# GAP-LAB-CUHK-SZ/GaussReg

Hardware: AMD Instinct MI355X
Metric: GS views/sec @1M pts 640x480 (+ radius_neighbors Mpts/sec, see radius_neighbors) (higher is better)
Workload: dtype f32; 1 GPU; diff_gaussian_rasterization forward: 1000000 synthetic Gaussians (SH deg 3), 640x480, 32 views per step per GPU (configs[1]); gaussians=1000000, width=640, height=480, parallelism=per-view sharding x1

## Files before the change

### gaussreg_amd/_lib.py

```python
import ctypes
import os
import re

_HERE = os.path.dirname(os.path.abspath(__file__))
LIB_PATH = os.path.join(_HERE, "lib", "libgaussreg_hip.so")
HEADER_PATH = os.path.join(_HERE, "..", "include", "gaussreg_hip.h")
TRAIN_HEADER_PATH = os.path.join(_HERE, "..", "include", "gaussreg_hip_train.h")
MATCH_TRAIN_HEADER_PATH = os.path.join(_HERE, "..", "include", "gaussreg_hip_train_matching.h")
BACKBONE_TRAIN_HEADER_PATH = os.path.join(_HERE, "..", "include", "gaussreg_hip_train_backbone.h")
CLOUD_HEADER_PATH = os.path.join(_HERE, "..", "include", "gaussreg_hip_cloud.h")
ICP_HEADER_PATH = os.path.join(_HERE, "..", "include", "gaussreg_hip_icp.h")

_lib = None

c_void = ctypes.c_void_p
c_f32 = ctypes.c_float


class RasterView(ctypes.Structure):
    _fields_ = [("image_height", ctypes.c_int32), ("image_width", ctypes.c_int32),
                ("tanfovx", c_f32), ("tanfovy", c_f32), ("bg", c_f32 * 3), ("scale_modifier", c_f32),
                ("viewmatrix", c_f32 * 16), ("projmatrix", c_f32 * 16), ("campos", c_f32 * 3),
                ("sh_degree", ctypes.c_int32), ("prefiltered", ctypes.c_int32), ("debug", ctypes.c_int32)]


class GsAdamGroup(ctypes.Structure):
    _fields_ = [("param", c_void), ("grad", c_void), ("exp_avg", c_void), ("exp_avg_sq", c_void),
                ("lr", ctypes.c_double), ("K", ctypes.c_int32)]


class GsDensifyGroup(ctypes.Structure):
    _fields_ = [("src_param", c_void), ("dst_param", c_void), ("src_exp_avg", c_void), ("dst_exp_avg", c_void),
                ("src_exp_avg_sq", c_void), ("dst_exp_avg_sq", c_void), ("K", ctypes.c_int32), ("role", ctypes.c_int32)]


_SCALARS = {"int": ctypes.c_int, "int32_t": ctypes.c_int32, "uint32_t": ctypes.c_uint32, "int64_t": ctypes.c_int64,
            "size_t": ctypes.c_size_t, "float": ctypes.c_float, "double": ctypes.c_double}
_POINTEES = set(_SCALARS) | {"void", "uint8_t", "uint64_t"}
_STRUCTS = {"gr_raster_view": RasterView, "gr_gs_adam_group": GsAdamGroup, "gr_gs_densify_group": GsDensifyGroup}
_TYPE = r"(?:const\s+)?(\w+)"


def _ctype(base, star, where):
    if star:
        if base == "char":
            return ctypes.c_char_p
        if base in _STRUCTS:
            return ctypes.POINTER(_STRUCTS[base])
        if base in _POINTEES:
            return ctypes.c_void_p
    elif base in _SCALARS:
        return _SCALARS[base]
    raise ValueError(f"gaussreg_hip.h: type '{base}{star}' in {where} is outside the binding's vocabulary")


def parse_header(text):
    text = re.sub(r"/\*.*?\*/", " ", text, flags=re.S)
    defines = {m.group(1): int(m.group(2)) for m in re.finditer(r"^[ \t]*#[ \t]*define[ \t]+(GR_\w+)[ \t]+(-?\d+)[ \t]*$",
                                                                  text, flags=re.M)}
    text = re.sub(r"^[ \t]*#.*$", "", text, flags=re.M)
    text = re.sub(r"\b(?:typedef\s+struct|enum)\b[^{};]*\{[^{}]*\}[^;]*;", "", text)
    text = re.sub(r'extern\s+"C"\s*\{(.*)\}', r"\1", text, flags=re.S)
    signatures = {}
    for decl in filter(None, (" ".join(d.split()) for d in text.split(";"))):
        m = re.fullmatch(r"(.+?)\b(gr_\w+) ?\((.*)\)", decl)
        if m is None:
            raise ValueError(f"gaussreg_hip.h: cannot parse the declaration '{decl}'")
        ret, name, args = m.group(1).strip(), m.group(2), m.group(3).strip()
        r = re.fullmatch(_TYPE + r"\s*(\*?)", ret)
        if r is None:
            raise ValueError(f"gaussreg_hip.h: cannot parse the return type '{ret}' of {name}")
        restype = None if r.groups() == ("void", "") else _ctype(r.group(1), r.group(2), f"the return type of {name}")
        argtypes = []
        for arg in ([] if args in ("", "void") else args.split(",")):
            a = re.fullmatch(_TYPE + r"(?:\s*(\*)\s*|\s+)\w+", arg.strip())
            if a is None:
                raise ValueError(f"gaussreg_hip.h: cannot parse the argument '{arg.strip()}' of {name}")
            argtypes.append(_ctype(a.group(1), a.group(2) or "", f"argument '{arg.strip()}' of {name}"))
        if name in signatures:
            raise ValueError(f"gaussreg_hip.h: {name} is declared twice")
        signatures[name] = (restype, argtypes)
    return signatures, defines


with open(HEADER_PATH) as _f:
    SIGNATURES, DEFINES = parse_header(_f.read())
with open(TRAIN_HEADER_PATH) as _f:
    TRAIN_SIGNATURES, TRAIN_DEFINES = parse_header(_f.read())
with open(MATCH_TRAIN_HEADER_PATH) as _f:
    MATCH_TRAIN_SIGNATURES, MATCH_TRAIN_DEFINES = parse_header(_f.read())
with open(BACKBONE_TRAIN_HEADER_PATH) as _f:
    BACKBONE_TRAIN_SIGNATURES, BACKBONE_TRAIN_DEFINES = parse_header(_f.read())
with open(CLOUD_HEADER_PATH) as _f:
    CLOUD_SIGNATURES, CLOUD_DEFINES = parse_header(_f.read())
with open(ICP_HEADER_PATH) as _f:
    ICP_SIGNATURES, ICP_DEFINES = parse_header(_f.read())

GR_PENDING = DEFINES["GR_PENDING"]
GR_RETRY_FULL = DEFINES["GR_RETRY_FULL"]
GR_RETRY_BIN = DEFINES["GR_RETRY_BIN"]
GS_ADAM_MAX_GROUPS = DEFINES["GR_GS_ADAM_MAX_GROUPS"]
GS_KNN_MAX_K = DEFINES["GR_GS_KNN_MAX_K"]
CLOUD_KNN_MAX_K = CLOUD_DEFINES["GR_CLOUD_KNN_MAX_K"]
CLOUD_ICP_MAX_ITERATIONS = ICP_DEFINES["GR_CLOUD_ICP_MAX_ITERATIONS"]
GS_DENSIFY_CARRIED, GS_DENSIFY_XYZ, GS_DENSIFY_SCALING = (DEFINES["GR_GS_DENSIFY_" + r] for r in ("CARRIED", "XYZ", "SCALING"))


class HipLibraryError(RuntimeError):
    pass


def lib():
    global _lib
    if _lib is None:
        import torch
        if not os.path.exists(LIB_PATH):
            raise HipLibraryError(
                f"{LIB_PATH} is missing: build it with `python -m gaussreg_amd.build` "
                "(there is no CPU fallback for the gaussreg_amd ops)")
        L = ctypes.CDLL(LIB_PATH)
        for name, (res, args) in (list(SIGNATURES.items()) + list(TRAIN_SIGNATURES.items())
                                   + list(MATCH_TRAIN_SIGNATURES.items()) + list(BACKBONE_TRAIN_SIGNATURES.items())
                                   + list(CLOUD_SIGNATURES.items()) + list(ICP_SIGNATURES.items())):
            fn = getattr(L, name)
            fn.restype = res
            fn.argtypes = args
        _lib = L
    return _lib


def check(rc, allow=()):
    if rc != 0 and rc not in allow:
        msg = lib().gr_last_error()
        raise RuntimeError("gaussreg_hip: " + (msg.decode() if msg else f"error {rc}"))
    return rc


def tensor_stamp(tensors):
    out = []
    for t in tensors:
        if t.is_inference():
            return None
        out.append((t.data_ptr(), t._version))
    return tuple(out)


def require_gpu():
    import torch
    if not torch.cuda.is_available():
        raise HipLibraryError("gaussreg_amd ops need an MI355X (torch.cuda.is_available() is False); "
                              "there is no CPU fallback")
    return torch.device("cuda", torch.cuda.current_device())


_ws_cache = {}


def workspace(device, nbytes):
    import threading

    import torch
    key = (device.type, device.index, torch.cuda.current_stream(device).cuda_stream, threading.get_ident())
    buf = _ws_cache.get(key)
    if buf is None or buf.numel() < nbytes:
        buf = torch.empty(int(nbytes * 1.25) + 4096, dtype=torch.uint8, device=device)
        _ws_cache[key] = buf
    return buf


def stream_ptr(device):
    import torch
    return ctypes.c_void_p(torch.cuda.current_stream(device).cuda_stream)


def ptr(t):
    return ctypes.c_void_p(t.data_ptr()) if t is not None else ctypes.c_void_p(0)
# ... 57 lines not shown
```

### gaussreg_amd/build.py

```python
import concurrent.futures
import os
import subprocess
import sys

HERE = os.path.dirname(os.path.abspath(__file__))
CSRC = os.path.join(HERE, "csrc")
LIBDIR = os.path.join(HERE, "lib")
OBJDIR = os.path.join(LIBDIR, "obj")
LIB = os.path.join(LIBDIR, "libgaussreg_hip.so")

HIPCC = os.environ.get("HIPCC", "/opt/rocm/bin/hipcc")
FLAGS = ["--offload-arch=gfx950", "-O3", "-std=c++17", "-fPIC", "-ffp-contract=off", "-Wall",
         "-Wno-unused-function", "-Wno-unused-result"]


def sources():
    return sorted(f for f in os.listdir(CSRC) if f.endswith(".hip"))


def _stale(out, deps):
    if not os.path.exists(out):
        return True
    t = os.path.getmtime(out)
    return any(os.path.getmtime(d) > t for d in deps)


def build(force=False, verbose=False):
    os.makedirs(OBJDIR, exist_ok=True)
    headers = [os.path.join(CSRC, f) for f in os.listdir(CSRC) if f.endswith((".hpp", ".h"))]
    headers += [os.path.join(HERE, "..", "include", h) for h in ("gaussreg_hip.h", "gaussreg_hip_train.h",
                                                                 "gaussreg_hip_train_matching.h",
                                                                 "gaussreg_hip_train_backbone.h", "gaussreg_hip_cloud.h",
                                                                 "gaussreg_hip_icp.h")]
    jobs = []
    objs = []
    for src in sources():
        s = os.path.join(CSRC, src)
        o = os.path.join(OBJDIR, src[:-4] + ".o")
        objs.append(o)
        if force or _stale(o, [s] + headers):
            jobs.append([HIPCC] + FLAGS + ["-c", s, "-o", o])

    def run(cmd):
        if verbose:
            print(" ".join(cmd), flush=True)
        r = subprocess.run(cmd, stdout=subprocess.PIPE, stderr=subprocess.STDOUT, text=True)
        return cmd, r.returncode, r.stdout

    if jobs:
        with concurrent.futures.ThreadPoolExecutor(max_workers=min(8, len(jobs))) as ex:
            for cmd, rc, out in ex.map(run, jobs):
                if rc != 0:
                    raise RuntimeError("hipcc failed: %s\n%s" % (" ".join(cmd), out))
                if verbose and out.strip():
                    print(out)
    if force or jobs or _stale(LIB, objs):
        cmd = [HIPCC, "--offload-arch=gfx950", "-shared", "-fPIC", "-o", LIB] + objs
        _, rc, out = run(cmd)
        if rc != 0:
            raise RuntimeError("link failed:\n" + out)
    return LIB


if __name__ == "__main__":
    print(build(force="--force" in sys.argv, verbose=True))
```

### gaussreg_amd/csrc/rasterizer.hip

```cpp
#include <algorithm>
#include <type_traits>
#include <vector>

#include <atomic>

#include "raster_shared.hpp"

namespace gr {
namespace {

static_assert(TILE == RASTER_TILE, "get_rect / rect_decode (common.hpp) are written for this tile size");


constexpr int KEY_DEPTH_BITS = 27;
constexpr uint32_t KEY_DEPTH_BASE = 0x3E000000u;

__device__ __forceinline__ uint32_t pack_rect(const int* rmin, const int* rmax) {
  const int w = rmax[0] - rmin[0], h = rmax[1] - rmin[1];
  if (w > 63 || h > 63 || rmin[0] > 126 || rmin[1] > 126) return RECT_MARKER26;
  return (uint32_t)rmin[0] | ((uint32_t)rmin[1] << 7) | ((uint32_t)w << 14) | ((uint32_t)h << 20);
}

constexpr int REC_PLANE = 66;
constexpr int SH_ROW = 13;

template <bool HAS_SH, bool HAS_COV, bool SH16, bool LATE>
__global__ __launch_bounds__(256) void preprocess_kernel(
    int P, int D, int M, int V, const DevView* __restrict__ views, const float* __restrict__ means3D,
    const float* __restrict__ shs, const float* __restrict__ colors_precomp,
    const float* __restrict__ opacities, const float* __restrict__ scales,
    const float* __restrict__ rotations, const float* __restrict__ cov3D_precomp, int W, int H,
    int32_t* __restrict__ radii, float4* __restrict__ rec, uint32_t* __restrict__ dfield,
    uint32_t* __restrict__ rect_raw, int32_t* __restrict__ far_flag, DevView cam1, int far_seq,
    int2* __restrict__ key_mm) {
  constexpr bool WAVE_MM = false;
#define GR_PREPROCESS_BODY_OK
#include "preprocess_body.hpp"
#undef GR_PREPROCESS_BODY_OK
}

template <bool HAS_SH, bool HAS_COV, bool SH16>
__global__ __launch_bounds__(256) void preprocess_many_kernel(
    int P, int D, int M, int V, const DevView* __restrict__ views, const float* __restrict__ means3D,
    const float* __restrict__ shs, const float* __restrict__ colors_precomp,
    const float* __restrict__ opacities, const float* __restrict__ scales,
    const float* __restrict__ rotations, const float* __restrict__ cov3D_precomp, int W, int H,
    int32_t* __restrict__ radii, float4* __restrict__ rec, uint32_t* __restrict__ dfield,
    uint32_t* __restrict__ rect_raw, int32_t* __restrict__ far_flag, DevView cam1, int far_seq,
    int2* __restrict__ key_mm) {
  constexpr bool WAVE_MM = true;
  constexpr bool LATE = false;
#define GR_PREPROCESS_BODY_OK
#include "preprocess_body.hpp"
#undef GR_PREPROCESS_BODY_OK
}

__global__ __launch_bounds__(256) void full_keys_kernel(int64_t n, const float4* __restrict__ rec,
                                                        const int32_t* __restrict__ radii, uint32_t* __restrict__ dfield) {
  const int64_t o = (int64_t)blockIdx.x * blockDim.x + threadIdx.x;
// ... 262 lines not shown
      int sum = 0, mx = 0;
      for (int i = threadIdx.x; i < nchunk; i += TT) {
        const int t = self.chunk_total[v * nchunk + i];
        sum += t;
        mx = max(mx, t);
      }
      sum = wave_sum_i32_dpp(sum);
      mx = wave_max_i32_dpp(mx);
      if (lane == 0) s_red[0][wv] = sum, s_red[1][wv] = mx;
      __syncthreads();
      if (threadIdx.x == 0) {
        int tv = 0, mv = 0;
        for (int w2 = 0; w2 < TT / WAVE; ++w2) tv += s_red[0][w2], mv = max(mv, s_red[1][w2]);
        self.totals[v] = tv;
        self.totals[V + v] = mv;
        if (self.mail != nullptr) {
          __hip_atomic_store(&self.mail[v], tv, __ATOMIC_RELAXED, __HIP_MEMORY_SCOPE_SYSTEM);
          __hip_atomic_store(&self.mail[V + v], mv, __ATOMIC_RELAXED, __HIP_MEMORY_SCOPE_SYSTEM);
          if (v == 0) __hip_atomic_store(&self.mail[2 * V], self.totals[2 * V], __ATOMIC_RELAXED, __HIP_MEMORY_SCOPE_SYSTEM);
          __hip_atomic_store(&self.mail[2 * V + 1 + v], self.mail_seq, __ATOMIC_RELEASE, __HIP_MEMORY_SCOPE_SYSTEM);
        }
      }
    }
  } else if (SEG == SEG_SELF_SCAN) {
    unsigned int front = (unsigned int)self.chunk_total[(int64_t)V * nchunk + v * nchunk + c];
    for (int u = 0; u < v; ++u) front += (unsigned int)self.totals[u];
    chunk_begin = front;
    total = self.chunk_total[v * nchunk + c];
  } else {
    chunk_begin = seg[0];
    total = (int)(seg[tiles] - chunk_begin);
    if (total == 0 || seg[tiles] > list_cap) return;
  }
  if (SELF && total == 0) {
    for (int T = threadIdx.x; T <= tiles; T += TT) seg[T] = chunk_begin;
    return;
  }
  const bool big = total > 0xffff;
  const bool staged = !big && total <= stage_cap;
  unsigned int* myw = s_cur + wv * (row / 2);
  unsigned short* const cur16 = reinterpret_cast<unsigned short*>(s_cur);
  unsigned short* my16 = cur16 + wv * row;
  unsigned short* stage = reinterpret_cast<unsigned short*>(s_cur + NW * (row / 2));
  unsigned int* elist = s_cur + NW * (row / 2) + (stage_cap + 1) / 2 + wv * elist_cap;
  for (int T = threadIdx.x; T < NW * (row / 2); T += TT) s_cur[T] = 0u;
  __syncthreads();
  const int w_end = min(nv, w_begin + CW);
#pragma unroll
  for (int j = 0; j < CW / WAVE; ++j) {
    const int t = w_begin + j * WAVE + lane;
    rr[j] = t < w_end ? rr[j] : 0u;
    ii[j] = t < w_end ? ii[j] : 0;
  }
  auto count = [&](int tile) { atomicAdd(&myw[tile >> 1], 1u << ((tile & 1) * 16)); };
#pragma unroll
  for (int j = 0; j < CW / WAVE; ++j) {
    const uint32_t r = rr[j];
    int x0 = 0, y0 = 0, w = 0, h = 0;
    if (r != 0u && !rect_decode(r, ii[j], vbase, rec, gx, gy, x0, y0, w, h)) w = h = 0;
    const int Mx = wave_max_i32_dpp(w), My = wave_max_i32_dpp(h);
    auto cwalk = [&](auto mtag) {
      constexpr int MX = decltype(mtag)::value;
      const int x0m = mod_small(x0, MX), y0m = mod_small(y0, My);
#pragma unroll 1
      for (int ry = 0; ry < My; ++ry) {
        int dy = ry - y0m;
        dy += dy < 0 ? My : 0;
        const int rowbase = (y0 + dy) * gx + x0;
#pragma unroll
        for (int rx = 0; rx < MX; ++rx) {
          int dx = rx - x0m;
          dx += dx < 0 ? MX : 0;
          if (dy < h && dx < w) count(rowbase + dx);
        }
      }
    };
    if (Mx == 0) continue;
    if (TT == WIDE_T || max(Mx, My) > 8) {
      for (int y = y0; y < y0 + h; ++y)
        for (int x = x0; x < x0 + w; ++x) count(y * gx + x);
    } else
      by_modulus(Mx, cwalk);
  }
  __syncthreads();
  if (SELF) {
    if (threadIdx.x == 0) s_carry = 0u;
    __syncthreads();
    for (int T0 = 0; T0 < tiles; T0 += TT) {
      const int T = T0 + (int)threadIdx.x;
      unsigned int cw[NW];
      int n_all = 0;
#pragma unroll
      for (int w2 = 0; w2 < NW; ++w2) {
        cw[w2] = T < tiles ? cur16[w2 * row + T] : 0u;
        n_all += (int)cw[w2];
      }
      const int incl = wave_incl_scan_add_dpp(n_all);
      if (lane == WAVE - 1) s_red[0][wv] = incl;
      __syncthreads();
      unsigned int before = s_carry + (unsigned int)(incl - n_all);
      for (int w2 = 0; w2 < wv; ++w2) before += (unsigned int)s_red[0][w2];
      if (T < tiles) {
        seg[T] = chunk_begin + before;
        unsigned int run = big ? 0u : before;
#pragma unroll
        for (int w2 = 0; w2 < NW; ++w2) {
          cur16[w2 * row + T] = (unsigned short)run;
          run += cw[w2];
        }
      }
      __syncthreads();
      if (threadIdx.x == TT - 1) s_carry = before + (unsigned int)n_all;
      __syncthreads();
    }
    if (threadIdx.x == 0) seg[tiles] = chunk_begin + (unsigned int)total;
    if (chunk_begin + (unsigned int)total > list_cap) return;
  } else {
    for (int T = threadIdx.x; T < tiles; T += TT) {
      unsigned int run = big ? 0u : seg[T] - chunk_begin;
#pragma unroll
      for (int w2 = 0; w2 < NW; ++w2) {
        const unsigned int n = cur16[w2 * row + T];
        cur16[w2 * row + T] = (unsigned short)run;
        run += n;
      }
    }
  }
  __syncthreads();
  auto put = [&](unsigned int tile, unsigned int pos, int local, int val) {
    if (staged) stage[pos] = (unsigned short)local;
    else if (!big) point_list[chunk_begin + pos] = val;
    else point_list[seg[tile] + pos] = val;
  };
  auto bump_raw = [&](unsigned int tile) -> unsigned int {
    return atomicAdd(&myw[tile >> 1], 1u << ((tile & 1u) * 16u));
// ... 547 lines not shown

int upload_views(const gr_raster_view* h_views, int num_views, int32_t* d_flag, hipStream_t stream) {
  static_assert(sizeof(DevView) % 4 == 0, "DevView is copied word by word");
  if (num_views <= VIEW_PACK) {
    ViewPack pack;
    memset(&pack, 0, sizeof(pack));
    for (int v = 0; v < num_views; ++v) fill_view(pack.v[v], h_views[v]);
    hipLaunchKernelGGL(upload_views_kernel, dim3(1), dim3(WAVE), 0, stream, pack, num_views, d_flag);
    GR_LAUNCH_CHECK();
    return GR_OK;
  }
  char* raw = static_cast<char*>(pinned_scratch(0, 16 + sizeof(DevView) * num_views));
  GR_REQUIRE(raw != nullptr, "pinned staging buffer for %d views could not be allocated", num_views);
  memset(raw, 0, 16);
  DevView* stage = reinterpret_cast<DevView*>(raw + 16);
  for (int v = 0; v < num_views; ++v) fill_view(stage[v], h_views[v]);
  GR_HIP(hipMemcpyAsync(d_flag, raw, 16 + sizeof(DevView) * num_views, hipMemcpyHostToDevice, stream));
  return GR_OK;
}

}
}

using namespace gr;

static int64_t tiles_of(int width, int height) {
  return (int64_t)((width + TILE - 1) / TILE) * ((height + TILE - 1) / TILE);
}

extern "C" int gr_raster_lds_atomics_lane_ordered(void) { return lds_atomics_lane_ordered_state(); }
extern "C" int gr_raster_ballot_ranking(int on) { return lds_ballot_ranking_force(on); }

extern "C" size_t gr_raster_geom_bytes(int64_t P, int num_views, int width, int height) {
  if (P < 0 || num_views < 1 || width <= 0 || height <= 0) return 0;
  return carve_geom(nullptr, P, num_views, tiles_of(width, height)).bytes;
}

extern "C" int gr_raster_debug_geom_layout(int64_t P, int num_views, int width, int height, int64_t* h_offsets) {
  GR_REQUIRE(P >= 0 && num_views >= 1 && width > 0 && height > 0 && h_offsets != nullptr, "bad argument");
  char* const origin = reinterpret_cast<char*>(uintptr_t(1) << 32);
  const Geom g = carve_geom(origin, P, num_views, tiles_of(width, height));
  h_offsets[0] = reinterpret_cast<char*>(g.dfield) - origin;
  h_offsets[1] = reinterpret_cast<char*>(g.order_b) - origin;
  h_offsets[2] = reinterpret_cast<char*>(g.rects) - origin;
  h_offsets[3] = reinterpret_cast<char*>(g.nvis) - origin;
  return 4;
}

extern "C" size_t gr_raster_bin_bytes(int64_t total_rendered, int width, int height, int num_views) {
  if (total_rendered < 0 || width <= 0 || height <= 0 || num_views < 1) return 0;
  return carve_bin(nullptr, total_rendered, tiles_of(width, height) * num_views).bytes;
}

struct Deferred {
  hipEvent_t ev;
  volatile int32_t* mail;
  int seq;
  int far_seq;
  bool by_mail;
  bool bucket_sort;
  bool self_seg;
};

static int preprocess_impl(int64_t P, int M, const float* means3D, const float* shs,
                           const float* colors_precomp, const float* opacities,
                           const float* scales, const float* rotations,
                           const float* cov3D_precomp, const gr_raster_view* h_views,
                           int num_views, int32_t* radii, void* geom, size_t geom_bytes,
                           int64_t* h_num_rendered, hipStream_t stream, Deferred* defer_ev) {
  int rc = check_views(h_views, num_views);
  if (rc != GR_OK) return rc;
  GR_REQUIRE(h_num_rendered != nullptr, "h_num_rendered is null");
  for (int v = 0; v <= num_views; ++v) h_num_rendered[v] = 0;
  GR_REQUIRE(P >= 0 && P < (1ll << 31) - 1, "P out of range");
  if (P == 0) {
    Geom g0 = carve_geom(geom, 0, num_views, tiles_of(h_views[0].image_width, h_views[0].image_height));
    if (!geom || geom_bytes < g0.bytes) {
      set_error("raster geometry buffer too small: need %zu bytes, got %zu", g0.bytes, geom_bytes);
      return GR_ERR_WORKSPACE;
    }
    rc = upload_views(h_views, num_views, g0.totals + 2 * num_views, stream);
    if (rc != GR_OK) return rc;
    GR_HIP(hipStreamSynchronize(stream));
    return GR_OK;
  }
  GR_REQUIRE(means3D && opacities && radii, "means3D / opacities / radii must be non-null");
  GR_REQUIRE((shs != nullptr) != (colors_precomp != nullptr),
             "Please provide excatly one of either SHs or precomputed colors!");
  GR_REQUIRE(((scales != nullptr && rotations != nullptr) != (cov3D_precomp != nullptr)) &&
                 ((scales != nullptr) == (rotations != nullptr)),
             "Please provide exactly one of either scale/rotation pair or precomputed 3D covariance!");
  const int D = h_views[0].sh_degree;
  if (shs) GR_REQUIRE(M >= (D + 1) * (D + 1), "shs has %d coefficients, sh_degree %d needs %d", M, D, (D + 1) * (D + 1));
  const int W = h_views[0].image_width, H = h_views[0].image_height;
  const int gx = (W + TILE - 1) / TILE, gy = (H + TILE - 1) / TILE;
  const int tiles = gx * gy;
  GR_REQUIRE(gx <= 255 && gy <= 255, "image too large: at most 255 x 255 tiles of 16 px (got %d x %d)", gx, gy);
  const size_t bin_lds = (size_t)(BIN_T / WAVE) * tiles * sizeof(unsigned int);
  GR_REQUIRE(bin_lds <= 156 * 1024, "image too large: the per-wave tile cursors (%zu bytes) do not fit in LDS", bin_lds);
  Geom g = carve_geom(geom, P, num_views, tiles);
  if (!geom || geom_bytes < g.bytes) {
    set_error("raster geometry buffer too small: need %zu bytes, got %zu", g.bytes, geom_bytes);
    return GR_ERR_WORKSPACE;
  }
  const dim3 blk(256), grd((unsigned)((P + 255) / 256));
  const bool sh16 = shs != nullptr && M == 16 && (reinterpret_cast<uintptr_t>(shs) % 16 == 0);
  const bool cam_in_args = sh16 && num_views == 1 && defer_ev != nullptr && defer_ev->mail != nullptr &&
                           (P + BIN_CHUNK - 1) / BIN_CHUNK <= SCAN_SINGLE_ROW;
  DevView cam1;
  memset(&cam1, 0, sizeof(cam1));
  int far_seq = 1;
  if (sh16 && num_views == 1) fill_view(cam1, h_views[0]);
  if (cam_in_args) {
    far_seq = defer_ev->seq;
  } else {
    rc = upload_views(h_views, num_views, g.totals + 2 * num_views, stream);
    if (rc != GR_OK) return rc;
  }
  if (defer_ev != nullptr) defer_ev->far_seq = far_seq;
  const bool msd_possible = depth_sort_msd_possible(P, num_views, KEY_DEPTH_BITS);
  const bool msd = msd_possible && (defer_ev != nullptr ? defer_ev->bucket_sort : bucket_sort_allowed(true));
  int2* const mm_out = msd ? g.key_mm : nullptr;
#define GR_PRE(SH, COV, S16)                                                                       \
  if (S16 && num_views == 1)                                                                       \
    hipLaunchKernelGGL((preprocess_kernel<SH, COV, S16, S16>), grd, blk, 0, stream, (int)P, D, M, num_views, \
                       g.views, means3D, shs, colors_precomp, opacities, scales, rotations,        \
                       cov3D_precomp, W, H, radii, g.rec, g.dfield, g.rect_raw, g.totals + 2 * num_views, cam1, far_seq, \
                       mm_out);                                                                    \
  else if (msd && num_views > 4)                                                                   \
    hipLaunchKernelGGL((preprocess_many_kernel<SH, COV, S16>), grd, blk, 0, stream, (int)P, D, M, num_views, \
                       g.views, means3D, shs, colors_precomp, opacities, scales, rotations,        \
                       cov3D_precomp, W, H, radii, g.rec, g.dfield, g.rect_raw, g.totals + 2 * num_views, cam1, far_seq, \
                       mm_out);                                                                    \
  else                                                                                             \
  hipLaunchKernelGGL((preprocess_kernel<SH, COV, S16, false>), grd, blk, 0, stream, (int)P, D, M, num_views, \
                     g.views, means3D, shs, colors_precomp, opacities, scales, rotations,          \
                     cov3D_precomp, W, H, radii, g.rec, g.dfield, g.rect_raw, g.totals + 2 * num_views, cam1, far_seq, \
                     mm_out)
  auto run_preprocess = [&]() {
    KernelTimer timer("raster_preprocess", stream);
    if (shs && cov3D_precomp) { if (sh16) GR_PRE(true, true, true); else GR_PRE(true, true, false); }
    else if (shs) { if (sh16) GR_PRE(true, false, true); else GR_PRE(true, false, false); }
    else if (cov3D_precomp) GR_PRE(false, true, false);
    else GR_PRE(false, false, false);
  };
  run_preprocess();
  GR_LAUNCH_CHECK();
  int32_t* tot = static_cast<int32_t*>(pinned_scratch(1, sizeof(int32_t) * (2 * num_views + 2)));
  GR_REQUIRE(tot != nullptr, "pinned read-back buffer could not be allocated");
  const int nchunk = (int)((P + BIN_CHUNK - 1) / BIN_CHUNK);
  int32_t h_chunk_max = 0;
  auto sort_and_count = [&](int key_bits, bool buckets = true) -> int {
    bool totals_sorted = false;
    {
      KernelTimer timer("raster_depth_sort", stream);
      const bool msd_now = msd && buckets && key_bits == KEY_DEPTH_BITS;
      const bool self_seg = msd_now && defer_ev != nullptr && defer_ev->mail != nullptr && nchunk <= SCAN_SINGLE_ROW &&
                            num_views <= 4;
      totals_sorted = msd_now && num_views > 4;
      const DepthSortTotals ct{g.chunk_total, BIN_CHUNK, nchunk, g.rec, gx, gy};
      int rcs = depth_sort_views(g.dfield, g.rect_raw, g.keys_a, g.keys_b, g.order_b, g.rects, g.nvis, P, num_views, key_bits,
                                 g.ds_table, g.ds_table_bytes, stream, msd_now ? g.key_mm : nullptr,
                                 num_views > 4 ? (int)((P + 255) / 256) * (256 / WAVE) : (int)((P + 255) / 256),
                                 g.totals + 2 * num_views, defer_ev != nullptr ? -far_seq : 2,
                                 self_seg || totals_sorted ? &ct : nullptr);
      if (rcs != GR_OK) return rcs;
      if (self_seg) {
        defer_ev->by_mail = true;
        defer_ev->self_seg = true;
        return GR_OK;
      }
    }
    {
      KernelTimer timer("raster_bin", stream);
      const bool short_rows = nchunk <= SCAN_SINGLE_ROW;
      if (!bin_scans_self(nchunk, num_views)) {
        if (tiles * sizeof(unsigned int) > 64 * 1024)
          GR_HIP(hipFuncSetAttribute(reinterpret_cast<const void*>(tile_count_kernel),
                                     hipFuncAttributeMaxDynamicSharedMemorySize, 160 * 1024));
        hipLaunchKernelGGL(tile_count_kernel, dim3((unsigned)bin_grid(num_views, nchunk)), dim3(BIN_T),
                           tiles * sizeof(unsigned int), stream, (int)P, num_views, gx, gy, nchunk, g.nvis, g.rects, g.order_b,
                           g.rec, g.chunk_cnt, g.chunk_total);
        const bool by_mail = defer_ev != nullptr && defer_ev->mail != nullptr;
        hipLaunchKernelGGL(seg_scan_kernel<true>, dim3((unsigned)(num_views * nchunk)), blk, 0, stream, num_views, tiles, nchunk,
                           g.chunk_cnt, g.chunk_total, g.totals, g.seg_off, by_mail ? const_cast<int32_t*>(defer_ev->mail) : nullptr,
                           by_mail ? defer_ev->seq : 0);
        if (by_mail) defer_ev->by_mail = true;
        GR_LAUNCH_CHECK();
      } else {
        if (!totals_sorted)
          hipLaunchKernelGGL(chunk_total_kernel, dim3((unsigned)bin_grid(num_views, nchunk)), dim3(BIN_T), 0, stream, (int)P,
                             num_views, gx, gy, nchunk, g.nvis, g.rects, g.order_b, g.rec, g.chunk_total);
        if (!short_rows)
          hipLaunchKernelGGL(chunk_max_kernel, dim3(1), dim3(1024), 0, stream, num_views * nchunk, g.chunk_total, g.chunk_max);
        GR_LAUNCH_CHECK();
        int rcs = exclusive_scan_i32(g.chunk_total, g.chunk_total + (int64_t)num_views * nchunk, nchunk, num_views, nchunk,
                                     g.scan_ws, g.totals, stream, nullptr, short_rows ? g.totals + num_views : nullptr);
        if (rcs != GR_OK) return rcs;
      }
    }
    const bool short_rows = nchunk <= SCAN_SINGLE_ROW;
    if (defer_ev != nullptr) {
      if (defer_ev->by_mail) return GR_OK;
      static thread_local hipStream_t side = nullptr;
      static thread_local hipEvent_t counted = nullptr;
      if (side == nullptr) GR_HIP(hipStreamCreateWithFlags(&side, hipStreamNonBlocking));
      if (counted == nullptr) GR_HIP(hipEventCreateWithFlags(&counted, hipEventDisableTiming));
      GR_HIP(hipEventRecord(counted, stream));
      GR_HIP(hipStreamWaitEvent(side, counted, 0));
      GR_HIP(hipMemcpyAsync(tot, g.totals, sizeof(int32_t) * (2 * num_views + 1), hipMemcpyDeviceToHost, side));
      if (!short_rows)
        GR_HIP(hipMemcpyAsync(tot + 2 * num_views + 1, g.chunk_max, sizeof(int32_t), hipMemcpyDeviceToHost, side));
      GR_HIP(hipEventRecord(defer_ev->ev, side));
      return GR_OK;
    }
    GR_HIP(hipMemcpyAsync(tot, g.totals, sizeof(int32_t) * (2 * num_views + 1), hipMemcpyDeviceToHost, stream));
    if (!short_rows)
      GR_HIP(hipMemcpyAsync(tot + 2 * num_views + 1, g.chunk_max, sizeof(int32_t), hipMemcpyDeviceToHost, stream));
    GR_HIP(hipStreamSynchronize(stream));
    h_chunk_max = short_rows ? tot[num_views] : tot[2 * num_views + 1];
    if (short_rows)
      for (int v = 1; v < num_views; ++v) h_chunk_max = std::max(h_chunk_max, tot[num_views + v]);
    return GR_OK;
  };
  rc = sort_and_count(KEY_DEPTH_BITS);
  if (rc != GR_OK) return rc;
  if (defer_ev != nullptr) return GR_OK;
  auto check_depth_order = [&]() -> int {
    if (!verify_this_frame()) return GR_OK;
    int h_bad = 0;
    int rcv = device_check(stream, [&](int* d_bad) {
      hipLaunchKernelGGL(verify_depth_order_kernel, dim3((unsigned)std::min<int64_t>((P + 255) / 256, 4096), num_views), blk, 0,
                         stream, (int)P, num_views, g.nvis, g.dfield, g.order_b, reinterpret_cast<int32_t*>(g.keys_a), d_bad);
    }, &h_bad);
    if (rcv != GR_OK) return rcv;
    if (h_bad != 0 && lds_atomics_lane_ordered_state() == 1) {
      lds_order_demote();
      return 1;
    }
    GR_REQUIRE(h_bad == 0, "depth sort produced an unsorted order (internal error)");
    return GR_OK;
  };
  if (tot[2 * num_views] & 2) {
    bucket_sort_overflowed();
    GR_HIP(hipMemsetD32Async(reinterpret_cast<hipDeviceptr_t>(g.totals + 2 * num_views), tot[2 * num_views] & 1, 1, stream));
    rc = sort_and_count(KEY_DEPTH_BITS, false);
    if (rc != GR_OK) return rc;
  }
  if (tot[2 * num_views] != 0) {
    hipLaunchKernelGGL(full_keys_kernel, dim3((unsigned)((P * num_views + 255) / 256)), blk, 0, stream, P * num_views,
                       g.rec, radii, g.dfield);
    GR_LAUNCH_CHECK();
    rc = sort_and_count(32);
    if (rc != GR_OK) return rc;
  }
  rc = check_depth_order();
  if (rc == 1) {
    rc = sort_and_count(tot[2 * num_views] != 0 ? 32 : KEY_DEPTH_BITS, false);
    if (rc != GR_OK) return rc;
    rc = check_depth_order();
// ... 165 lines not shown
  hipLaunchKernelGGL((blend_kernel<FE, KEEP>), dim3(gx, gy, num_views), dim3(BLOCK), blend_pad, stream, (int)P, W, H,      \
                     blend_chunks, g.views, g.seg_off, point_list, g.rec, out_color, list_cap, BlendAux<false>{})
#define GR_BLEND_AUX(FE, KEEP)                                                                                        \
  hipLaunchKernelGGL((blend_kernel<FE, KEEP, true>), dim3(gx, gy, num_views), dim3(BLOCK), 0, stream, (int)P, W, H,        \
                     blend_chunks, g.views, g.seg_off, point_list, g.rec, out_color, list_cap,                           \
                     BlendAux<true>{out_depth, out_alpha, aux_state})
  if (out_depth != nullptr) {
    if (keep) { if (fast) GR_BLEND_AUX(true, true); else GR_BLEND_AUX(false, true); }
    else if (fast) GR_BLEND_AUX(true, false); else GR_BLEND_AUX(false, false);
  }
  else if (keep) { if (fast) GR_BLEND(true, true); else GR_BLEND(false, true); }
  else if (fast) GR_BLEND(true, false); else GR_BLEND(false, false);
#undef GR_BLEND
#undef GR_BLEND_AUX
  GR_LAUNCH_CHECK();
  frame_done();
  return GR_OK;
}

extern "C" int gr_raster_render_ex(int64_t P, const gr_raster_view* h_views, int num_views,
                                   const int64_t* h_num_rendered, const void* geom, size_t geom_bytes,
                                   void* bin, size_t bin_bytes, float* out_color, int flags, void* stream_) {
  return render_impl(P, h_views, num_views, h_num_rendered, geom, geom_bytes, bin, bin_bytes, out_color, flags, -1,
                     static_cast<hipStream_t>(stream_));
}

extern "C" int gr_raster_render_keep(int64_t P, const gr_raster_view* h_views, int num_views,
                                     const int64_t* h_num_rendered, const void* geom, size_t geom_bytes,
                                     void* bin, size_t bin_bytes, float* out_state, int flags, void* stream_) {
  return render_impl(P, h_views, num_views, h_num_rendered, geom, geom_bytes, bin, bin_bytes, out_state, flags, -1,
                     static_cast<hipStream_t>(stream_), nullptr, true);
}

extern "C" int gr_raster_render_aux(int64_t P, const gr_raster_view* h_views, int num_views,
                                    const int64_t* h_num_rendered, const void* geom, size_t geom_bytes,
                                    void* bin, size_t bin_bytes, float* out_color, float* out_depth, float* out_alpha,
                                    float* out_state, int flags, void* stream_) {
  GR_REQUIRE(out_depth != nullptr && out_alpha != nullptr, "out_depth / out_alpha is null");
  return render_impl(P, h_views, num_views, h_num_rendered, geom, geom_bytes, bin, bin_bytes, out_color, flags, -1,
                     static_cast<hipStream_t>(stream_), nullptr, out_state != nullptr, out_depth, out_alpha, out_state);
}

namespace gr {
namespace {
struct Pending {
  bool open;
  int64_t P;
  int num_views;
  int64_t entries;
  Deferred d;
  hipStream_t stream;
};
thread_local Pending g_pending{false, 0, 0, 0, Deferred{nullptr, nullptr, 0, 0, false, false, false}, nullptr};
}
}

extern "C" int gr_raster_debug_bucket_cooldown(int set) {
  const int left = gr::g_bucket_cooldown;
  if (set >= 0) gr::g_bucket_cooldown = set;
  return left;
}

extern "C" int gr_raster_forward_finish(int64_t* h_num_rendered) {
  using namespace gr;
  GR_REQUIRE(g_pending.open, "gr_raster_forward_finish: no split gr_raster_forward is open on this thread");
  GR_REQUIRE(h_num_rendered != nullptr, "h_num_rendered is null");
  Pending p = g_pending;
  g_pending.open = false;
  bool far_depth = false, bucket_overflow = false;
  int rc = preprocess_collect(p.P, p.num_views, h_num_rendered, &far_depth, p.d, p.stream, &bucket_overflow);
  if (rc != GR_OK) return rc;
  if (bucket_overflow) bucket_sort_overflowed();
  int64_t R = 0;
  for (int v = 0; v < p.num_views; ++v) R += h_num_rendered[v];
  if (far_depth) return GR_RETRY_FULL;
  return R <= p.entries ? GR_OK : GR_RETRY_BIN;
}

extern "C" int gr_raster_forward(int64_t P, int M, const float* means3D, const float* shs, const float* colors_precomp,
                                 const float* opacities, const float* scales, const float* rotations,
                                 const float* cov3D_precomp, const gr_raster_view* h_views, int num_views, int32_t* radii,
                                 void* geom, size_t geom_bytes, void* bin, size_t bin_bytes, float* out_color, int flags,
                                 int64_t* h_num_rendered, void* stream_) {
  hipStream_t stream = static_cast<hipStream_t>(stream_);
  GR_REQUIRE(h_num_rendered != nullptr, "h_num_rendered is null");
  GR_REQUIRE(!g_pending.open, "gr_raster_forward: the previous split call of this thread was not finished");
  const int64_t stage_hint = h_num_rendered[num_views > 0 ? num_views : 0];
  const int64_t entries = bin && bin_bytes > 512 ? (int64_t)((bin_bytes - 512) / sizeof(int32_t)) - 64 : -1;
  if (P > 0 && num_views <= 4 && entries > 0 && entries < (1ll << 31) - 1 && !verify_this_frame()) {
    static thread_local hipEvent_t ev = nullptr;
    if (ev == nullptr) GR_HIP(hipEventCreateWithFlags(&ev, hipEventDisableTiming));
    static thread_local int32_t* mail = nullptr;
    if (mail == nullptr) {
      static const bool no_mail = getenv("GR_NO_MAILBOX") && getenv("GR_NO_MAILBOX")[0] == '1';
      void* mp = nullptr;
      if (!no_mail && hipHostMalloc(&mp, 4096, hipHostMallocMapped | hipHostMallocCoherent) == hipSuccess) {
        memset(mp, 0, 4096);
        mail = static_cast<int32_t*>(mp);
      } else {
        (void)hipGetLastError();
      }
    }
    static std::atomic<int> frame_seq{0};
    int seq = frame_seq.fetch_add(1) + 1;
    if (seq > 0x7ffffff0) {
      frame_seq.store(1);
      seq = 1;
    }
    Deferred d{ev, mail, seq, 1, false, bucket_sort_allowed(depth_sort_msd_possible(P, num_views, KEY_DEPTH_BITS)), false};
    int rc = preprocess_impl(P, M, means3D, shs, colors_precomp, opacities, scales, rotations, cov3D_precomp, h_views,
                             num_views, radii, geom, geom_bytes, h_num_rendered, stream, &d);
    if (rc != GR_OK) return rc;
    h_num_rendered[num_views] = stage_hint;
    rc = render_impl(P, h_views, num_views, h_num_rendered, geom, geom_bytes, bin, bin_bytes, out_color, flags, entries, stream,
                     &d);
    if (rc != GR_OK) return rc;
    if (flags & GR_RASTER_SPLIT) {
      g_pending = Pending{true, P, num_views, entries, d, stream};
      return GR_PENDING;
    }
    bool far_depth = false, bucket_overflow = false;
    rc = preprocess_collect(P, num_views, h_num_rendered, &far_depth, d, stream, &bucket_overflow);
    if (rc != GR_OK) return rc;
    if (bucket_overflow) bucket_sort_overflowed();
    int64_t R = 0;
    for (int v = 0; v < num_views; ++v) R += h_num_rendered[v];
    if (!far_depth) return R <= entries ? GR_OK : GR_RETRY_BIN;
  }
  int rc = gr_raster_preprocess(P, M, means3D, shs, colors_precomp, opacities, scales, rotations, cov3D_precomp, h_views,
                                num_views, radii, geom, geom_bytes, h_num_rendered, stream);
  if (rc != GR_OK) return rc;
  int64_t R = 0;
  for (int v = 0; v < num_views; ++v) R += h_num_rendered[v];
  if (bin == nullptr || bin_bytes < gr_raster_bin_bytes(R, h_views[0].image_width, h_views[0].image_height, num_views))
    return GR_RETRY_BIN;
  return gr_raster_render_ex(P, h_views, num_views, h_num_rendered, geom, geom_bytes, bin, bin_bytes, out_color, flags, stream);
}

extern "C" int gr_raster_mark_visible(int64_t P, const float* means3D, const float* h_viewmatrix,
                                      uint8_t* present, void* stream_) {
  hipStream_t stream = static_cast<hipStream_t>(stream_);
  GR_REQUIRE(P >= 0 && h_viewmatrix != nullptr, "bad argument");
  if (P == 0) return GR_OK;
  GR_REQUIRE(means3D && present, "null argument");
  hipLaunchKernelGGL(mark_visible_kernel, dim3((unsigned)((P + 255) / 256)), dim3(256), 0, stream, (int)P, means3D,
                     h_viewmatrix[2], h_viewmatrix[6], h_viewmatrix[10], h_viewmatrix[14], present);
  GR_LAUNCH_CHECK();
  return GR_OK;
}
```

Measured before the change: 14160 views/s.

## Extend speculative single-sync forward path to batches of more than four views

```diff
diff --git a/gaussreg_amd/_lib.py b/gaussreg_amd/_lib.py
--- a/gaussreg_amd/_lib.py
+++ b/gaussreg_amd/_lib.py
@@ -10,6 +10,7 @@
 BACKBONE_TRAIN_HEADER_PATH = os.path.join(_HERE, "..", "include", "gaussreg_hip_train_backbone.h")
 CLOUD_HEADER_PATH = os.path.join(_HERE, "..", "include", "gaussreg_hip_cloud.h")
 ICP_HEADER_PATH = os.path.join(_HERE, "..", "include", "gaussreg_hip_icp.h")
+RASTER_DEBUG_HEADER_PATH = os.path.join(_HERE, "..", "include", "gaussreg_hip_raster_debug.h")
 
 _lib = None
 
@@ -95,6 +96,8 @@
     CLOUD_SIGNATURES, CLOUD_DEFINES = parse_header(_f.read())
 with open(ICP_HEADER_PATH) as _f:
     ICP_SIGNATURES, ICP_DEFINES = parse_header(_f.read())
+with open(RASTER_DEBUG_HEADER_PATH) as _f:
+    RASTER_DEBUG_SIGNATURES, RASTER_DEBUG_DEFINES = parse_header(_f.read())
 
 GR_PENDING = DEFINES["GR_PENDING"]
 GR_RETRY_FULL = DEFINES["GR_RETRY_FULL"]
@@ -121,7 +124,8 @@
         L = ctypes.CDLL(LIB_PATH)
         for name, (res, args) in (list(SIGNATURES.items()) + list(TRAIN_SIGNATURES.items())
                                    + list(MATCH_TRAIN_SIGNATURES.items()) + list(BACKBONE_TRAIN_SIGNATURES.items())
-                                   + list(CLOUD_SIGNATURES.items()) + list(ICP_SIGNATURES.items())):
+                                   + list(CLOUD_SIGNATURES.items()) + list(ICP_SIGNATURES.items())
+                                   + list(RASTER_DEBUG_SIGNATURES.items())):
             fn = getattr(L, name)
             fn.restype = res
             fn.argtypes = args
diff --git a/gaussreg_amd/build.py b/gaussreg_amd/build.py
--- a/gaussreg_amd/build.py
+++ b/gaussreg_amd/build.py
@@ -31,7 +31,7 @@
     headers += [os.path.join(HERE, "..", "include", h) for h in ("gaussreg_hip.h", "gaussreg_hip_train.h",
                                                                  "gaussreg_hip_train_matching.h",
                                                                  "gaussreg_hip_train_backbone.h", "gaussreg_hip_cloud.h",
-                                                                 "gaussreg_hip_icp.h")]
+                                                                 "gaussreg_hip_icp.h", "gaussreg_hip_raster_debug.h")]
     jobs = []
     objs = []
     for src in sources():
diff --git a/gaussreg_amd/csrc/rasterizer.hip b/gaussreg_amd/csrc/rasterizer.hip
--- a/gaussreg_amd/csrc/rasterizer.hip
+++ b/gaussreg_amd/csrc/rasterizer.hip
@@ -5,6 +5,7 @@
 #include <atomic>
 
 #include "raster_shared.hpp"
+#include "../../include/gaussreg_hip_raster_debug.h"
 
 namespace gr {
 namespace {
@@ -1055,6 +1056,16 @@
   return carve_bin(nullptr, total_rendered, tiles_of(width, height) * num_views).bytes;
 }
 
+static int count_readback_stream(hipStream_t* side_out, hipEvent_t* counted_out) {
+  static thread_local hipStream_t side = nullptr;
+  static thread_local hipEvent_t counted = nullptr;
+  if (side == nullptr) GR_HIP(hipStreamCreateWithFlags(&side, hipStreamNonBlocking));
+  if (counted == nullptr) GR_HIP(hipEventCreateWithFlags(&counted, hipEventDisableTiming));
+  *side_out = side;
+  *counted_out = counted;
+  return GR_OK;
+}
+
 struct Deferred {
   hipEvent_t ev;
   volatile int32_t* mail;
@@ -1070,7 +1081,7 @@
                            const float* scales, const float* rotations,
                            const float* cov3D_precomp, const gr_raster_view* h_views,
                            int num_views, int32_t* radii, void* geom, size_t geom_bytes,
-                           int64_t* h_num_rendered, hipStream_t stream, Deferred* defer_ev) {
+                           int64_t* h_num_rendered, hipStream_t stream, Deferred* defer_ev, int bucket_choice = -1) {
   int rc = check_views(h_views, num_views);
   if (rc != GR_OK) return rc;
   GR_REQUIRE(h_num_rendered != nullptr, "h_num_rendered is null");
@@ -1122,7 +1133,8 @@
   }
   if (defer_ev != nullptr) defer_ev->far_seq = far_seq;
   const bool msd_possible = depth_sort_msd_possible(P, num_views, KEY_DEPTH_BITS);
-  const bool msd = msd_possible && (defer_ev != nullptr ? defer_ev->bucket_sort : bucket_sort_allowed(true));
+  const bool msd = msd_possible && (defer_ev != nullptr ? defer_ev->bucket_sort
+                                    : bucket_choice >= 0 ? bucket_choice != 0 : bucket_sort_allowed(true));
   int2* const mm_out = msd ? g.key_mm : nullptr;
 #define GR_PRE(SH, COV, S16)                                                                       \
   if (S16 && num_views == 1)                                                                       \
@@ -1205,10 +1217,10 @@
     const bool short_rows = nchunk <= SCAN_SINGLE_ROW;
     if (defer_ev != nullptr) {
       if (defer_ev->by_mail) return GR_OK;
-      static thread_local hipStream_t side = nullptr;
-      static thread_local hipEvent_t counted = nullptr;
-      if (side == nullptr) GR_HIP(hipStreamCreateWithFlags(&side, hipStreamNonBlocking));
-      if (counted == nullptr) GR_HIP(hipEventCreateWithFlags(&counted, hipEventDisableTiming));
+      hipStream_t side = nullptr;
+      hipEvent_t counted = nullptr;
+      int rce = count_readback_stream(&side, &counted);
+      if (rce != GR_OK) return rce;
       GR_HIP(hipEventRecord(counted, stream));
       GR_HIP(hipStreamWaitEvent(side, counted, 0));
       GR_HIP(hipMemcpyAsync(tot, g.totals, sizeof(int32_t) * (2 * num_views + 1), hipMemcpyDeviceToHost, side));
@@ -1480,7 +1492,19 @@
   hipStream_t stream;
 };
 thread_local Pending g_pending{false, 0, 0, 0, Deferred{nullptr, nullptr, 0, 0, false, false, false}, nullptr};
-}
+
+thread_local int g_spec_backoff = 0;
+constexpr int SPEC_BACKOFF_CALLS = 256;
+thread_local int g_forward_path = GR_RASTER_PATH_PLAIN;
+}
+}
+
+extern "C" int gr_raster_debug_forward_path(void) { return gr::g_forward_path; }
+
+extern "C" int gr_raster_debug_spec_backoff(int set) {
+  const int left = gr::g_spec_backoff;
+  if (set >= 0) gr::g_spec_backoff = set;
+  return left;
 }
 
 extern "C" int gr_raster_debug_bucket_cooldown(int set) {
@@ -1501,6 +1525,7 @@
   if (bucket_overflow) bucket_sort_overflowed();
   int64_t R = 0;
   for (int v = 0; v < p.num_views; ++v) R += h_num_rendered[v];
+  if (far_depth && p.num_views > 4) g_spec_backoff = SPEC_BACKOFF_CALLS;
   if (far_depth) return GR_RETRY_FULL;
   return R <= p.entries ? GR_OK : GR_RETRY_BIN;
 }
@@ -1515,7 +1540,29 @@
   GR_REQUIRE(!g_pending.open, "gr_raster_forward: the previous split call of this thread was not finished");
   const int64_t stage_hint = h_num_rendered[num_views > 0 ? num_views : 0];
   const int64_t entries = bin && bin_bytes > 512 ? (int64_t)((bin_bytes - 512) / sizeof(int32_t)) - 64 : -1;
-  if (P > 0 && num_views <= 4 && entries > 0 && entries < (1ll << 31) - 1 && !verify_this_frame()) {
+  const bool many = num_views > 4;
+  if (many && P > 0 && geom != nullptr && geom_bytes >= sizeof(int32_t)) {
+    static thread_local bool warmed = false;
+    if (!warmed) {
+      hipStream_t side = nullptr;
+      hipEvent_t counted = nullptr;
+      int rcw = count_readback_stream(&side, &counted);
+      if (rcw != GR_OK) return rcw;
+      void* tot = pinned_scratch(1, sizeof(int32_t) * (2 * num_views + 2));
+      GR_REQUIRE(tot != nullptr, "pinned read-back buffer could not be allocated");
+      GR_HIP(hipMemcpyAsync(tot, geom, sizeof(int32_t), hipMemcpyDeviceToHost, side));
+      GR_HIP(hipStreamSynchronize(side));
+      warmed = true;
+    }
+  }
+  bool speculate = P > 0 && entries > 0 && entries < (1ll << 31) - 1 && !verify_this_frame();
+  if (many && P > 0 && g_spec_backoff > 0) {
+    --g_spec_backoff;
+    speculate = false;
+  }
+  g_forward_path = GR_RASTER_PATH_PLAIN;
+  int bucket_choice = -1;
+  if (speculate) {
     static thread_local hipEvent_t ev = nullptr;
     if (ev == nullptr) GR_HIP(hipEventCreateWithFlags(&ev, hipEventDisableTiming));
     static thread_local int32_t* mail = nullptr;
@@ -1535,7 +1582,8 @@
       frame_seq.store(1);
       seq = 1;
     }
-    Deferred d{ev, mail, seq, 1, false, bucket_sort_allowed(depth_sort_msd_possible(P, num_views, KEY_DEPTH_BITS)), false};
+    Deferred d{ev, many ? nullptr : mail, seq, 1, false,
+               bucket_sort_allowed(depth_sort_msd_possible(P, num_views, KEY_DEPTH_BITS)), false};
     int rc = preprocess_impl(P, M, means3D, shs, colors_precomp, opacities, scales, rotations, cov3D_precomp, h_views,
                              num_views, radii, geom, geom_bytes, h_num_rendered, stream, &d);
     if (rc != GR_OK) return rc;
@@ -1543,6 +1591,7 @@
     rc = render_impl(P, h_views, num_views, h_num_rendered, geom, geom_bytes, bin, bin_bytes, out_color, flags, entries, stream,
                      &d);
     if (rc != GR_OK) return rc;
+    g_forward_path = d.by_mail ? GR_RASTER_PATH_MAIL : GR_RASTER_PATH_EVENT;
     if (flags & GR_RASTER_SPLIT) {
       g_pending = Pending{true, P, num_views, entries, d, stream};
       return GR_PENDING;
@@ -1554,9 +1603,14 @@
     int64_t R = 0;
     for (int v = 0; v < num_views; ++v) R += h_num_rendered[v];
     if (!far_depth) return R <= entries ? GR_OK : GR_RETRY_BIN;
-  }
-  int rc = gr_raster_preprocess(P, M, means3D, shs, colors_precomp, opacities, scales, rotations, cov3D_precomp, h_views,
-                                num_views, radii, geom, geom_bytes, h_num_rendered, stream);
+    g_forward_path = GR_RASTER_PATH_REDONE;
+    if (many) {
+      g_spec_backoff = SPEC_BACKOFF_CALLS;
+      bucket_choice = d.bucket_sort && !bucket_overflow ? 1 : 0;
+    }
+  }
+  int rc = preprocess_impl(P, M, means3D, shs, colors_precomp, opacities, scales, rotations, cov3D_precomp, h_views, num_views,
+                           radii, geom, geom_bytes, h_num_rendered, stream, nullptr, bucket_choice);
   if (rc != GR_OK) return rc;
   int64_t R = 0;
   for (int v = 0; v < num_views; ++v) R += h_num_rendered[v];
diff --git a/include/gaussreg_hip_raster_debug.h b/include/gaussreg_hip_raster_debug.h
--- /dev/null
+++ b/include/gaussreg_hip_raster_debug.h
@@ -0,0 +1,19 @@
+#ifndef GAUSSREG_HIP_RASTER_DEBUG_H_
+#define GAUSSREG_HIP_RASTER_DEBUG_H_
+
+#ifdef __cplusplus
+extern "C" {
+#endif
+
+#define GR_RASTER_PATH_PLAIN 0
+#define GR_RASTER_PATH_EVENT 1
+#define GR_RASTER_PATH_MAIL 2
+#define GR_RASTER_PATH_REDONE 3
+int gr_raster_debug_forward_path(void);
+int gr_raster_debug_spec_backoff(int set);
+
+#ifdef __cplusplus
+}
+#endif
+
+#endif
```

Result: no change. 14200 views/s, median of 6 (+0.3%).

## Count tile overlaps with 2D difference array and prefix sums instead of per-tile atomics

Applied to the files above, without the earlier changes.

```diff
diff --git a/gaussreg_amd/csrc/rasterizer.hip b/gaussreg_amd/csrc/rasterizer.hip
--- a/gaussreg_amd/csrc/rasterizer.hip
+++ b/gaussreg_amd/csrc/rasterizer.hip
@@ -373,35 +373,91 @@
     rr[j] = t < w_end ? rr[j] : 0u;
     ii[j] = t < w_end ? ii[j] : 0;
   }
-  auto count = [&](int tile) { atomicAdd(&myw[tile >> 1], 1u << ((tile & 1) * 16)); };
-#pragma unroll
-  for (int j = 0; j < CW / WAVE; ++j) {
-    const uint32_t r = rr[j];
-    int x0 = 0, y0 = 0, w = 0, h = 0;
-    if (r != 0u && !rect_decode(r, ii[j], vbase, rec, gx, gy, x0, y0, w, h)) w = h = 0;
-    const int Mx = wave_max_i32_dpp(w), My = wave_max_i32_dpp(h);
-    auto cwalk = [&](auto mtag) {
-      constexpr int MX = decltype(mtag)::value;
-      const int x0m = mod_small(x0, MX), y0m = mod_small(y0, My);
-#pragma unroll 1
-      for (int ry = 0; ry < My; ++ry) {
-        int dy = ry - y0m;
-        dy += dy < 0 ? My : 0;
-        const int rowbase = (y0 + dy) * gx + x0;
-#pragma unroll
-        for (int rx = 0; rx < MX; ++rx) {
-          int dx = rx - x0m;
-          dx += dx < 0 ? MX : 0;
-          if (dy < h && dx < w) count(rowbase + dx);
-        }
-      }
-    };
-    if (Mx == 0) continue;
-    if (TT == WIDE_T || max(Mx, My) > 8) {
+  if constexpr (TT == WIDE_T) {
+    auto count = [&](int tile) { atomicAdd(&myw[tile >> 1], 1u << ((tile & 1) * 16)); };
+#pragma unroll
+    for (int j = 0; j < CW / WAVE; ++j) {
+      const uint32_t r = rr[j];
+      int x0 = 0, y0 = 0, w = 0, h = 0;
+      if (r != 0u && !rect_decode(r, ii[j], vbase, rec, gx, gy, x0, y0, w, h)) w = h = 0;
+      const int Mx = wave_max_i32_dpp(w);
+      if (Mx == 0) continue;
       for (int y = y0; y < y0 + h; ++y)
         for (int x = x0; x < x0 + w; ++x) count(y * gx + x);
-    } else
-      by_modulus(Mx, cwalk);
+    }
+  } else {
+    static_assert(CW <= 0x7fff, "signed 16-bit difference cells");
+    auto corner = [&](int tile, unsigned int one) { atomicAdd(&myw[tile >> 1], one << ((tile & 1) * 16)); };
+    auto wave_sync = [] {
+      __builtin_amdgcn_fence(__ATOMIC_RELEASE, "wavefront");
+      __builtin_amdgcn_wave_barrier();
+      __builtin_amdgcn_fence(__ATOMIC_ACQUIRE, "wavefront");
+    };
+#pragma unroll
+    for (int j = 0; j < CW / WAVE; ++j) {
+      const uint32_t r = rr[j];
+      int x0 = 0, y0 = 0, w = 0, h = 0;
+      if (r != 0u && rect_decode(r, ii[j], vbase, rec, gx, gy, x0, y0, w, h)) {
+        const int t00 = y0 * gx + x0, t10 = t00 + h * gx;
+        const bool in_x = x0 + w < gx, in_y = y0 + h < gy;
+        corner(t00, 1u);
+        if (in_x) corner(t00 + w, ~0u);
+        if (in_y) corner(t10, ~0u);
+        if (in_x && in_y) corner(t10 + w, 1u);
+      }
+    }
+    wave_sync();
+    if ((gx & 1) == 0) {
+      const int nw = gx >> 1;
+      for (int k = lane; k < nw; k += WAVE) {
+        unsigned int run = 0u;
+        int y = 0;
+        for (; y + 4 <= gy; y += 4) {
+          unsigned int* p = myw + y * nw + k;
+          const unsigned int a0 = p[0], a1 = p[nw], a2 = p[2 * nw], a3 = p[3 * nw];
+          p[0] = run += a0;
+          p[nw] = run += a1;
+          p[2 * nw] = run += a2;
+          p[3 * nw] = run += a3;
+        }
+        for (; y < gy; ++y) myw[y * nw + k] = run += myw[y * nw + k];
+      }
+      wave_sync();
+      for (int y = lane; y < gy; y += WAVE) {
+        unsigned int* p = myw + y * nw;
+        unsigned int front = 0u;
+        auto step = [&](unsigned int n) {
+          n += (n << 16) + front;
+          front = (n >> 16) * 0x10001u;
+          return n;
+        };
+        int k = 0;
+        for (; k + 4 <= nw; k += 4) {
+          const unsigned int a0 = p[k], a1 = p[k + 1], a2 = p[k + 2], a3 = p[k + 3];
+          p[k] = step(a0);
+          p[k + 1] = step(a1);
+          p[k + 2] = step(a2);
+          p[k + 3] = step(a3);
+        }
+        for (; k < nw; ++k) p[k] = step(p[k]);
+      }
+    } else {
+      for (int i = lane; i < row / 2; i += WAVE) {
+        const unsigned int n = myw[i];
+        myw[i] = n + ((n & 0x8000u) << 1);
+      }
+      wave_sync();
+      short* g16 = reinterpret_cast<short*>(my16);
+      for (int x = lane; x < gx; x += WAVE) {
+        int run = 0;
+        for (int y = 0; y < gy; ++y) g16[y * gx + x] = (short)(run += g16[y * gx + x]);
+      }
+      wave_sync();
+      for (int y = lane; y < gy; y += WAVE) {
+        int run = 0;
+        for (int x = 0; x < gx; ++x) g16[y * gx + x] = (short)(run += g16[y * gx + x]);
+      }
+    }
   }
   __syncthreads();
   if (SELF) {
```

New measurement: 14170 views/s before, 14360 views/s after (median of 6 runs). +1.4%, better.
